# omnirevolve/omnirevolve-image-processor

Measured on NVIDIA B200. Metric: megapixels/sec (resize+color+edge), higher is better.
Workload: dtype u8

## Files before the change

### omnirevolve-image-processor_b200/csrc/label_pipe.cu

```cuda
#include "fast_device.cuh"

#include <algorithm>
#include <vector>
#include <stdio.h>
#include <stdlib.h>
#include <string.h>

#define LP_ZBUF 8192
#define SP_TRY(expr) do { int rc__ = (expr); if (rc__ != OMNI_OK) return rc__; } while (0)


__global__ void __launch_bounds__(256) fk_permute_boxes3(const u8 *__restrict__ boxes, uint2 *__restrict__ boxes3)
{
    const int idx = blockIdx.x * blockDim.x + threadIdx.x;
    if (idx >= RC_COUNT) return;
    const int ci = ((idx & 63) << 12) | (((idx >> 6) & 63) << 6) | (idx >> 12);
    const u8 *q = boxes + 6 * ci;
    boxes3[idx] = make_uint2((u32)q[0] | ((u32)q[1] << 8) | ((u32)q[2] << 16) | ((u32)q[3] << 24), (u32)q[4] | ((u32)q[5] << 8));
}

__device__ __forceinline__ u32 lp_candidates(const AssignParams &P, const float (&lo)[3], const float (&hi)[3], bool &sane)
{
    const int K = P.K;
    float U = 3.0e38f;
// ... 170 lines not shown
            u32 t = nibw & (nibw >> 1) & (nibw >> 2) & (nibw >> 3) & 0x11111111u;
            t = (t | (t >> 3)) & 0x03030303u;
            mm = (t * 0x01041040u) >> 24;
        }
        if (!full) {
            const int nv = max(0, min(8, w - xbase));
            const u32 keep = nv >= 8 ? 0xffffffffu : ((1u << (4 * nv)) - 1u);
            nibw &= keep;
            mm &= (1u << nv) - 1u;
        }
        const int cnt = __popc(mm);
        int x = cnt;
#pragma unroll
        for (int d = 1; d < 32; d <<= 1) {
            int t = __shfl_up_sync(0xffffffffu, x, d);
            if (lane >= d) x += t;
        }
        const int nq = __shfl_sync(0xffffffffu, x, 31);
        if (nq) {
            int pos = x - cnt;
#pragma unroll
            for (int j = 0; j < 8; j++)
                if ((mm >> j) & 1u) sq[pos++] = (u8)(8 * lane + j);
            __syncwarp();
            for (int i = lane; i < nq; i += 32) {
                const int pi = sq[i];
                const u8 *p = spx + 3 * pi;
                int L, a, b, best = 0;
                lab_noclamp(s_gam, s_cbrt, p[0], p[1], p[2], L, a, b);
                u32 mk = __ldg(cells + (((L >> CELL_SHIFT) * CELL_N + (a >> CELL_SHIFT)) * CELL_N + (b >> CELL_SHIFT)));
                const float f0 = (float)L, f1 = (float)a, f2 = (float)b;
                float bd = 3.0e38f;
                do {
                    const int k = __ffs(mk) - 1;
                    mk &= mk - 1u;
                    const float4 ck = s_ctr[k];
                    float d0 = __fsub_rn(f0, ck.x), d1 = __fsub_rn(f1, ck.y), d2 = __fsub_rn(f2, ck.z);
                    float d = __fadd_rn(__fadd_rn(__fmul_rn(d0, d0), __fmul_rn(d1, d1)), __fmul_rn(d2, d2));
                    if (d < bd) { bd = d; best = k; }
                } while (mk);
                slab[pi] = s_lut[best];
            }
            __syncwarp();
            if (mm) {
                const uint2 lb = *reinterpret_cast<const uint2 *>(slab + 8 * lane);
                u32 t0 = lb.x & 0x0F0F0F0Fu, t1 = lb.y & 0x0F0F0F0Fu;
                t0 = (t0 | (t0 >> 4)) & 0x00FF00FFu; t0 = (t0 | (t0 >> 8)) & 0xFFFFu;
                t1 = (t1 | (t1 >> 4)) & 0x00FF00FFu; t1 = (t1 | (t1 >> 8)) & 0xFFFFu;
                const u32 fix = t0 | (t1 << 16);
                u32 m = mm;
                m = (m | (m << 12)) & 0x000F000Fu; m = (m | (m << 6)) & 0x03030303u; m = (m | (m << 3)) & 0x11111111u;
                m *= 15u;
                nibw = (nibw & ~m) | (fix & m);
            }
        }
        if (labels) {
            u32 b0 = nibw & 0xFFFFu, b1 = nibw >> 16;
            b0 = (b0 | (b0 << 8)) & 0x00FF00FFu; b0 = (b0 | (b0 << 4)) & 0x0F0F0F0Fu;
            b1 = (b1 | (b1 << 8)) & 0x00FF00FFu; b1 = (b1 | (b1 << 4)) & 0x0F0F0F0Fu;
            u8 *lrow = labels + (size_t)yy * lpitch + xbase;
            if (lab_vec && xbase + 8 <= w) *reinterpret_cast<uint2 *>(lrow) = make_uint2(b0, b1);
            else
                for (int j = 0; j < 8 && xbase + j < w; j++) lrow[j] = (u8)((nibw >> (4 * j)) & 15u);
        }
        {
            u32 r[4];
#pragma unroll
            for (int b = 0; b < 4; b++) {
                const u32 xb = (nibw >> b) & 0x11111111u;
                const u32 x1 = (xb | (xb >> 3)) & 0x03030303u;
                r[b] = x1 * 0x01041040u;
            }
            const u32 pk = __byte_perm(__byte_perm(r[0], r[1], 0x7373), __byte_perm(r[2], r[3], 0x7373), 0x5410);
            u32 t = __shfl_xor_sync(0xffffffffu, pk, 1);
            const u32 v1 = __byte_perm(pk, t, sel1);
            t = __shfl_xor_sync(0xffffffffu, v1, 2);
            const u32 word = __byte_perm(v1, t, sel2);
            if (c * 8 + (lane >> 2) < ws) slices[(((size_t)f * h + y) * ws + (size_t)c * 8) * 4 + lane] = word;
        }
    }
    if (lane == 0) asm volatile("cp.async.bulk.wait_group.read 0;" ::: "memory");
}

#define LO_WARPS 4
#define LP_COLS 30
#define LO_ROWS 8

__global__ void __launch_bounds__(LO_WARPS * 32) fk_label_open(const uint4 *__restrict__ slices, int ws, size_t plane, int h, int w, int nf,
                                                               u32 *__restrict__ od_out, int strips, int wcols)
{
    const int lane = threadIdx.x & 31;
    const long long gw = (long long)blockIdx.x * LO_WARPS + (threadIdx.x >> 5);
    const long long per_f = (long long)strips * wcols;
    if (gw >= per_f * nf) return;
    const int f = (int)(gw / per_f);
    const int rem = (int)(gw - (long long)f * per_f);
    const int strip = rem / wcols, wx = rem - strip * wcols;
    const int ww = (w + 31) >> 5;
    const int c = wx * LP_COLS - 1 + lane;
    const bool inimg = c >= 0 && c < ww;
    const bool owned = inimg && lane >= 1 && lane <= LP_COLS;
    const u32 cm = inimg ? range_mask(32 * c, w) : 0u;
    const u32 lfix = (c == 0) ? 1u : 0u;
    const u32 rfix = (c == ww - 1) ? (1u << ((w - 1) & 31)) : 0u;
    const uint4 *sl = slices + (size_t)f * plane;
    u32 *od = od_out + (size_t)f * plane;
    const int ys = strip * LO_ROWS, ye = min(h, ys + LO_ROWS);
    u32 sp[4] = {0u, 0u, 0u, 0u}, dh1 = 0u, dh2 = 0u, dv1 = 0u, hu2 = 0u, hu3 = 0u;
    u32 ns[4], ne[4];
    auto fetch = [&](const int r) {
        const bool rin = r >= 0 && r < h;
        uint4 v = make_uint4(0u, 0u, 0u, 0u), ev = v;
        if (rin) {
            const uint4 *row = sl + (size_t)r * ws;
            if (inimg) v = __ldg(row + c);
            if (lane == 0 && c - 1 >= 0 && c - 1 < ww) ev = __ldg(row + c - 1);
            if (lane == 31 && c + 1 >= 0 && c + 1 < ww) ev = __ldg(row + c + 1);
        }
        ns[0] = v.x; ns[1] = v.y; ns[2] = v.z; ns[3] = v.w;
        ne[0] = ev.x; ne[1] = ev.y; ne[2] = ev.z; ne[3] = ev.w;
    };
    fetch(ys - 2);
    for (int r = ys - 2; r < ye + 2; r++) {
        u32 s[4], e[4];
#pragma unroll
        for (int b = 0; b < 4; b++) { s[b] = ns[b]; e[b] = ne[b]; }
        fetch(r + 1);
        const bool rin = r >= 0 && r < h;
        u32 dl = 0u, dr = 0u, dv = 0u;
#pragma unroll
        for (int b = 0; b < 4; b++) {
            const u32 m = s[b];
            u32 l = __shfl_up_sync(0xffffffffu, m, 1), rr = __shfl_down_sync(0xffffffffu, m, 1);
            if (lane == 0) l = e[b];
            if (lane == 31) rr = e[b];
            dl |= m ^ __funnelshift_l(l, m, 1);
            dr |= m ^ __funnelshift_r(m, rr, 1);
            dv |= m ^ sp[b];
            sp[b] = m;
        }
        dl &= ~lfix; dr &= ~rfix;
        const u32 dh0 = rin ? (dl | dr) : 0u;
        const u32 dv0 = (rin && r > 0) ? dv : 0u;
        const bool yin = r - 1 >= 0 && r - 1 < h;
        const u32 U = yin ? (~(dh2 | dh1 | dh0 | dv1 | dv0) & cm) : 0u;
        const u32 l = __shfl_up_sync(0xffffffffu, U, 1), rr = __shfl_down_sync(0xffffffffu, U, 1);
        const u32 hu1 = U | __funnelshift_l(l, U, 1) | __funnelshift_r(U, rr, 1);
        const int z = r - 2;
        if (owned && z >= ys && z < ye) od[(size_t)z * ws + c] = (hu3 | hu2 | hu1) & cm;
        hu3 = hu2; hu2 = hu1; dh2 = dh1; dh1 = dh0; dv1 = dv0;
    }
}

template <int OP>
__device__ __forceinline__ u32 step32(const u32 u, const u32 m, const u32 d)
{
    if (OP == ST_ER || OP == ST_DR) {
        const u32 v = OP == ST_ER ? (u & m & d) : (u | m | d);
        const u32 l = __shfl_up_sync(0xffffffffu, v, 1), r = __shfl_down_sync(0xffffffffu, v, 1);
        const u32 sl = __funnelshift_l(l, v, 1), sr = __funnelshift_r(v, r, 1);
        return OP == ST_ER ? (v & sl & sr) : (v | sl | sr);
    }
    if (OP == ST_EC || OP == ST_DC) {
        const u32 l = __shfl_up_sync(0xffffffffu, m, 1), r = __shfl_down_sync(0xffffffffu, m, 1);
        const u32 sl = __funnelshift_l(l, m, 1), sr = __funnelshift_r(m, r, 1);
        return OP == ST_EC ? ((m & sl & sr) & u & d) : ((m | sl | sr) | u | d);
    }
    return m;
}

template <int NEXT, bool ROWFIX, bool COLFIX>
__device__ __forceinline__ u32 oob_fix32(u32 v, const u32 colvalid, const bool row_inside)
{
    if (NEXT == ST_NONE) return COLFIX ? (v & colvalid) : v;
    if (op_is_erode(NEXT)) {
        if (ROWFIX && !row_inside) return 0xffffffffu;
        return COLFIX ? (v | ~colvalid) : v;
    }
    if (ROWFIX && !row_inside) return 0u;
    return COLFIX ? (v & colvalid) : v;
}

template <u32 CODE, int S>
struct MorphChain32 {
    template <int TAP, bool ROWFIX, bool COLFIX>
    static __device__ __forceinline__ void run(u32 cur, u32 (&p1)[8], u32 (&p2)[8], int t, int h, u32 colvalid, u32 &tap_out, u32 &fin)
    {
        constexpr int N = code_len(CODE);
        if (S == TAP) tap_out = cur;
        if constexpr (S < N) {
            constexpr int OP = code_op(CODE, S);
            constexpr int NEXT = (S + 1 < N) ? code_op(CODE, S + 1) : ST_NONE;
            u32 out = step32<OP>(p2[S], p1[S], cur);
            p2[S] = p1[S]; p1[S] = cur;
            const int r = t - S - 1;
            out = oob_fix32<NEXT, ROWFIX, COLFIX>(out, colvalid, !ROWFIX || (r >= 0 && r < h));
            MorphChain32<CODE, S + 1>::template run<TAP, ROWFIX, COLFIX>(out, p1, p2, t, h, colvalid, tap_out, fin);
        } else {
            fin = cur;
        }
    }
};

#ifndef ML_ORDER
#define ML_ORDER 1
#endif
#ifndef ML_MINB
#define ML_MINB 1
#endif
template <u32 CODE, int TAP, int TR, bool RUNS>
__global__ void __launch_bounds__(128, ML_MINB) fk_morph_lab(const uint4 *__restrict__ slices, const u32 *__restrict__ od, u32 *__restrict__ out_bits, int ws,
                                                    size_t plane, int h, int w, int K, u8 *__restrict__ masks, size_t mstride, size_t mpitch,
                                                    int aligned16, u32 *__restrict__ tap_bits, int wcols, int strips, int n_planes, long long n_units,
                                                    const __grid_constant__ MorphRuns R)
{
    constexpr int N = code_len(CODE);
    constexpr int EXT = RUNS ? 2 : 0;
    constexpr int TILES = TR / ET_R;
    __shared__ uint2 s_lut8[256];
    __shared__ u32 s_item[4][TILES][32];
    expand_lut_init(s_lut8, threadIdx.x, blockDim.x);
    __syncthreads();
    const int lane = threadIdx.x & 31, wid = threadIdx.x >> 5;
    const long long unit = (long long)blockIdx.x * 4 + wid;
    if (unit >= n_units) return;
#if ML_ORDER == 3
    const int p = (int)(unit % n_planes);
    const long long u2 = unit / n_planes;
    const int wx = (int)(u2 % wcols), strip = (int)(u2 / wcols);
#else
    const int wx = (int)(unit % wcols);
    const long long u2 = unit / wcols;
#if ML_ORDER == 1
    const int p = (int)(u2 % n_planes), strip = (int)(u2 / n_planes);
#else
    const int strip = (int)(u2 % strips), p = (int)(u2 / strips);
#endif
#endif
    const int ww = (w + 31) >> 5;
    const int c = wx * LP_COLS - 1 + lane;
    const bool inimg = c >= 0 && c < ww;
    const bool owned = inimg && lane >= 1 && lane <= LP_COLS;
    const int f = p / K, k = p - f * K;
    const int y0 = strip * TR, y1 = min(h, y0 + TR);
    const int t_first = y0 - N - EXT;
    const uint4 *sl = slices + (ptrdiff_t)f * (ptrdiff_t)plane + (ptrdiff_t)t_first * ws + c;
    const u32 *odp = od + (ptrdiff_t)f * (ptrdiff_t)plane + (ptrdiff_t)t_first * ws + c;
    u8 *mrow = masks + (size_t)p * mstride + (ptrdiff_t)(t_first - TAP) * (ptrdiff_t)mpitch;
    u32 *trow = tap_bits + (ptrdiff_t)p * (ptrdiff_t)plane + (ptrdiff_t)(t_first - TAP) * ws + c;
    u32 *frow = out_bits + (ptrdiff_t)p * (ptrdiff_t)plane + (ptrdiff_t)(t_first - N) * ws + c;
    const u32 n0 = (k & 1) ? 0u : 0xffffffffu, n1 = (k & 2) ? 0u : 0xffffffffu, n2 = (k & 4) ? 0u : 0xffffffffu,
              n3 = (k & 8) ? 0u : 0xffffffffu;
    const u32 colvalid = inimg ? range_mask(32 * c, w) : 0u;
    const u32 lv = (c >= 1 && c <= ww) ? 0xC0000000u : 0u;
    const u32 rv = (c + 1 >= 0) ? (range_mask(32 * c + 32, w) & 3u) : 0u;
    constexpr int OP0 = code_op(CODE, 0);
    u32 p1[8], p2[8];
#pragma unroll
    for (int s = 0; s < 8; s++) p1[s] = p2[s] = 0u;
    uint4 nsl = make_uint4(0u, 0u, 0u, 0u);
    u32 nod = 0u;
    auto fetch = [&](const int t) {
        nod = 0u;
        if (t >= 0 && t < h && inimg) { nod = __ldg(odp); nsl = __ldg(sl); }
        odp += ws; sl += ws;
    };
    u32 live1 = 0u, live0 = 0u;
    auto rows = [&](auto rowfix_tag, auto colfix_tag) {
        constexpr bool ROWFIX = decltype(rowfix_tag)::value, COLFIX = decltype(colfix_tag)::value;
        fetch(t_first);
        for (int t = t_first; t < y1 + N + EXT; t++) {
            u32 cur = nod & (nsl.x ^ n0) & (nsl.y ^ n1) & (nsl.z ^ n2) & (nsl.w ^ n3);
            const bool inside = t >= 0 && t < h;
            fetch(t + 1);
            cur = oob_fix32<OP0, ROWFIX, COLFIX>(cur, colvalid, !ROWFIX || inside);
            u32 tap = 0u, fin = 0u;
            MorphChain32<CODE, 0>::template run<TAP, ROWFIX, COLFIX>(cur, p1, p2, t, h, colvalid, tap, fin);
            {
                const int r = t - TAP;
                if (r >= y0 && r < y1 && owned) {
                    if (masks) store_word_bytes_lut(mrow, 32 * c, w, tap, aligned16, s_lut8);
                    if (tap_bits) *trow = tap & colvalid;
                }
                mrow += mpitch; trow += ws;
            }
            if (!RUNS) continue;
            const int r = t - N;
            if (r >= y0 && r < y1 && owned) *frow = fin & colvalid;
            frow += ws;
            if (r >= y0 - 2 && r < y1 + 2 && (!ROWFIX || (r >= 0 && r < h))) {
                const u32 l = __shfl_up_sync(0xffffffffu, fin, 1), rr = __shfl_down_sync(0xffffffffu, fin, 1);
                const bool h1 = ((fin & colvalid) | (l & lv) | (rr & rv)) != 0u, h0 = ((~fin & colvalid) | (~l & lv) | (~rr & rv)) != 0u;
                const int q = r - y0, sub = q & 7;
                u32 m = 1u << ((q >> 3) + 1);
                if (sub < 2) m |= m >> 1;
                if (sub >= 6) m |= m << 1;
                m = (m >> 1) & ((1u << TILES) - 1u);
                if (h1) live1 |= m;
                if (h0) live0 |= m;
            }
        }
    };
    const bool rowfix = !(y0 - N - EXT >= 0 && y1 + N + EXT <= h);
    const bool colfix = __any_sync(0xffffffffu, colvalid != 0xffffffffu);
    if (rowfix) { if (colfix) rows(std::true_type{}, std::true_type{}); else rows(std::true_type{}, std::false_type{}); }
    else { if (colfix) rows(std::false_type{}, std::true_type{}); else rows(std::false_type{}, std::false_type{}); }
    if (!RUNS) return;
    const u32 live = owned ? (live1 & live0) : 0u;
    int n_items = 0, run = 0, run_j0 = 0;
    u32 lens = 0u;
    auto emit = [&]() {
        lens |= (u32)run << (3 * n_items);
        s_item[wid][n_items++][lane] = ((u32)p << 27) | ((u32)run_j0 << 13) | (u32)c;
        run = 0;
    };
#pragma unroll
    for (int tl = 0; tl < TILES; tl++) {
        const int ty0 = y0 + tl * ET_R;
        if (ty0 >= y1) break;
        if ((live >> tl) & 1u) {
            if (run == 0) run_j0 = ty0 / ET_R;
            if (++run == R.maxt) emit();
        } else {
            if (run) emit();
            if (owned && R.zero_fill) {
                const int ty1 = min(y1, ty0 + ET_R);
                for (int y = ty0; y < ty1; y++) {
                    const size_t o = (size_t)p * plane + (size_t)y * ws + c;
                    R.cbits[o] = 0u; R.sbits[o] = 0u;
                    if (R.edges) store_word_bytes(R.edges + (size_t)p * R.estride + (size_t)y * R.epitch, 32 * c, w, 0u, R.aligned16);
                }
            }
        }
    }
    if (run) emit();
#pragma unroll
    for (int nt = 1; nt <= ET_MAXT; nt++) {
        int mine = 0;
        for (int i = 0; i < n_items; i++) mine += ((lens >> (3 * i)) & 7u) == (u32)nt;
        int x = mine;
#pragma unroll
        for (int d = 1; d < 32; d <<= 1) {
            int y = __shfl_up_sync(0xffffffffu, x, d);
            if (lane >= d) x += y;
        }
        const int total = __shfl_sync(0xffffffffu, x, 31);
        if (total == 0) continue;
        int base = 0;
        if (lane == 31) base = atomicAdd(R.run_counts + nt - 1, total);
        base = __shfl_sync(0xffffffffu, base, 31);
        int pos = base + x - mine;
        for (int i = 0; i < n_items; i++)
            if (((lens >> (3 * i)) & 7u) == (u32)nt) R.run_items[R.off.v[nt - 1] + pos++] = s_item[wid][i][lane];
    }
}

#define WS5_LABEL_BYTES ((size_t)CELL_COUNT * sizeof(u32) + RC_NIB_BYTES + RC_MB_BYTES)

static int label_tables(omni_ctx *ctx, const AssignParams &P, u32 **cells, u8 **rtab, cudaStream_t st)
{
    SP_TRY(omni_ws_reserve(ctx, 5, WS5_BYTES + WS5_LABEL_BYTES));
    *cells = (u32 *)((u8 *)ctx->ws[5] + WS5_BYTES);
    *rtab = (u8 *)(*cells + CELL_COUNT);
    if ((ctx->table_cache || ctx->tables_hold) && ctx->cells3_valid && ctx->cells3_ws == ctx->ws[5] && ctx->cells3_stream == (void *)st && ctx->cells3_K == P.K &&
        memcmp(ctx->cells3_c, P.c, sizeof(float) * 3 * P.K) == 0 && memcmp(ctx->cells3_lut, P.lut, P.K) == 0)
        return OMNI_OK;
    memcpy(ctx->cells3_c, P.c, sizeof(float) * 3 * P.K);
    memcpy(ctx->cells3_lut, P.lut, P.K);
    ctx->cells3_K = P.K; ctx->cells3_stream = (void *)st; ctx->cells3_valid = 1; ctx->cells3_ws = ctx->ws[5];
    if (!ctx->d_rgb_boxes3) {
        SP_TRY(fast_rgb_boxes(ctx, st));
        OMNI_CUDA(cudaMalloc(&ctx->d_rgb_boxes3, (size_t)RC_COUNT * sizeof(uint2)));
        KScope ks(ctx, "rgb_boxes", st);
        fk_permute_boxes3<<<RC_COUNT / 256, 256, 0, st>>>(ctx->d_rgb_boxes, (uint2 *)ctx->d_rgb_boxes3);
        OMNI_CUDA(cudaGetLastError());
    }
    KScope ks(ctx, "build_tables", st);
    fk_build_tables3<<<LP_TAB_BLOCKS, 256, 0, st>>>(P, (const uint2 *)ctx->d_rgb_boxes3, *rtab, (u32 *)(*rtab + RC_NIB_BYTES), *cells);
    OMNI_CUDA(cudaGetLastError());
    return OMNI_OK;
}

constexpr u32 CODE_L_N = mk_code(ST_DR, ST_ER);
constexpr u32 CODE_L_O = mk_code(ST_DR, ST_ER, ST_EC, ST_DC);
constexpr u32 CODE_L_C = mk_code(ST_DR, ST_ER, ST_DC, ST_EC);
constexpr u32 CODE_L_OC = mk_code(ST_DR, ST_ER, ST_EC, ST_DC, ST_DC, ST_EC);

static cudaError_t launch_morph_lab(int kind , const uint4 *slices, const u32 *od, u32 *m2, const BitGeom &g, int K, int KT,
                                    u8 *masks, size_t mstride, size_t mpitch, u32 *tap_bits, const MorphRuns &R, cudaStream_t st)
{
    const int wcols = (g.ww + LP_COLS - 1) / LP_COLS;
    const int al = plane_align(masks, mstride, mpitch);
#ifdef ML_TR
    const int tr = ML_TR;
#else
    static int resident = 0;
    if (resident == 0) {
        int per_sm = 0, dev = 0, sms = 0;
        if (cudaOccupancyMaxActiveBlocksPerMultiprocessor(&per_sm, fk_morph_lab<CODE_L_OC, 2, 64, true>, 128, 0) != cudaSuccess || per_sm < 1) per_sm = 4;
        if (cudaGetDevice(&dev) != cudaSuccess || cudaDeviceGetAttribute(&sms, cudaDevAttrMultiProcessorCount, dev) != cudaSuccess || sms < 1) sms = 148;
        cudaGetLastError();
        resident = per_sm * 4 * sms;
    }
    int tr = 32;
    long long best = -1;
    for (int cand : {32, 56, 64}) {
        const long long units = (long long)wcols * ((g.h + cand - 1) / cand) * KT;
        const long long cost = ((units + resident - 1) / resident) * (cand + 20);
        if (best < 0 || cost <= best) { best = cost; tr = cand; }
    }
#endif
    const int strips = (g.h + tr - 1) / tr;
    const long long n_units = (long long)wcols * strips * KT;
    dim3 b(128), grid((unsigned)((n_units + 3) / 4));
#define LL2(CODE, TRV, RUNS) fk_morph_lab<CODE, 2, TRV, RUNS><<<grid, b, 0, st>>>(slices, od, m2, g.ws, g.plane, g.h, g.w, K, masks, mstride, mpitch, al, tap_bits, wcols, strips, KT, n_units, R)
#ifdef ML_TR
#define LL(CODE, RUNS) LL2(CODE, ML_TR, RUNS)
#else
#define LL(CODE, RUNS) do { if (tr == 64) LL2(CODE, 64, RUNS); else if (tr == 56) LL2(CODE, 56, RUNS); else LL2(CODE, 32, RUNS); } while (0)
#endif
    switch (kind) {
    case -1: LL(CODE_L_N, false); break;
    case 0: LL(CODE_L_N, true); break;
    case 1: LL(CODE_L_O, true); break;
    case 2: LL(CODE_L_C, true); break;
    default: LL(CODE_L_OC, true); break;
    }
#undef LL
#undef LL2
    return cudaGetLastError();
}

struct LabelPlanes { u32 *slices, *mask_bits, *edge_bits, *cand_bits; };

static int label_pipeline(omni_ctx *ctx, const u8 *d_bgr, int nf, size_t frame_stride, int h, int w, size_t pitch, const AssignParams &P,
                          const omni_edge_params *prm, int low, int high, u8 *d_labels, size_t lpitch,
                          u8 *d_masks, size_t m_plane, size_t mpitch, u8 *d_edges, size_t e_plane, size_t epitch, bool want_mask_bits,
                          cudaStream_t st, LabelPlanes *out, bool skip_hysteresis = false )
{
    const int K = P.K, KT = nf * K;
    const int kind = prm ? morph03_kind(prm) : -1;
    if (prm && (low < 0 || kind < 0 || prm->ksize != 3)) return OMNI_ERR_UNSUPPORTED;
    if (K > RC_MAX_K || KT > OMNI_MAX_K || !lut_below_k(P) || !edges3_sparse_ok(h, w, KT)) return OMNI_ERR_UNSUPPORTED;
    const BitGeom g = make_geom(h, w);
    if ((long long)nf * h * ((w + 255) >> 8) >= (1ll << 30)) return OMNI_ERR_UNSUPPORTED;
    OMNI_CUDA(fast_tables());
    const size_t pbytes = g.plane * sizeof(u32);
    auto al = [](size_t v) { return (v + 255) & ~(size_t)255; };
    const size_t o_sl = 0, o_od = al(o_sl + pbytes * 4 * nf), o_m2 = al(o_od + pbytes * nf), o_s = al(o_m2 + pbytes * KT),
                 o_c = o_s + al(pbytes * KT), o_mb = al(o_c + pbytes * KT), bits_total = al(o_mb + (want_mask_bits ? pbytes * KT : 0));
    SP_TRY(omni_ws_reserve(ctx, 4, bits_total));
    u8 *b4 = (u8 *)ctx->ws[4];
    u32 *slices = (u32 *)(b4 + o_sl), *od = (u32 *)(b4 + o_od), *M2 = (u32 *)(b4 + o_m2), *sbits = (u32 *)(b4 + o_s), *cbits = (u32 *)(b4 + o_c);
    u32 *mbits = want_mask_bits ? (u32 *)(b4 + o_mb) : nullptr;
    if (out) { out->slices = slices; out->mask_bits = mbits; out->edge_bits = prm ? sbits : nullptr; out->cand_bits = prm ? cbits : nullptr; }
    MorphRuns R{};
    bool sparse = false;
    ZeroJob Z{};
    if (prm) {
        SP_TRY(edge_pass_begin(ctx, g, KT, sbits, cbits, d_edges, e_plane, epitch, st, &R, &sparse, d_edges != nullptr, d_edges ? &Z : nullptr));
        if (!sparse) return OMNI_ERR_UNSUPPORTED;
    }
    u32 *cells = nullptr;
    u8 *rtab = nullptr;
    SP_TRY(label_tables(ctx, P, &cells, &rtab, st));
    const u16 *labtab = fast_lab_table();
    if (!labtab) { omni_set_error("Lab tables not available"); return OMNI_ERR_CUDA; }
    {
        if (!ctx->occ_assign_sl) {
            OMNI_CUDA(cudaFuncSetAttribute(fk_assign_slices<true>, cudaFuncAttributeMaxDynamicSharedMemorySize, RA_SMEM + LP_ZBUF));
            OMNI_CUDA(cudaFuncSetAttribute(fk_assign_slices<false>, cudaFuncAttributeMaxDynamicSharedMemorySize, RA_SMEM + LP_ZBUF));
            ctx->occ_assign_sl = 1;
        }
        const long long chunks = (long long)nf * h * ((w + 255) >> 8);
        const int grid = (int)std::max<long long>(1, std::min<long long>(persist_blocks(ctx, 1), (chunks + RA_WARPS - 1) / RA_WARPS));
        for (int z = 0; z < 2; z++)
            Z.per[z] = (unsigned)(((Z.n16[z] + (unsigned long long)chunks - 1) / (unsigned long long)chunks + 31) & ~31ull);
        KScope ks(ctx, "assign_bits", st);
        if (K >= 16)
            fk_assign_slices<true><<<grid, RA_THREADS, RA_SMEM + LP_ZBUF, st>>>(d_bgr, h, w, pitch, P, (const uint4 *)rtab, cells, labtab, d_labels,
                                                                                lpitch, slices, g.ws, nf, frame_stride, Z);
        else
            fk_assign_slices<false><<<grid, RA_THREADS, RA_SMEM + LP_ZBUF, st>>>(d_bgr, h, w, pitch, P, (const uint4 *)rtab, cells, labtab, d_labels,
                                                                                 lpitch, slices, g.ws, nf, frame_stride, Z);
        OMNI_CUDA(cudaGetLastError());
    }
    {
        const int wcols = (g.ww + LP_COLS - 1) / LP_COLS, strips = (h + LO_ROWS - 1) / LO_ROWS;
        const long long warps = (long long)nf * strips * wcols;
        KScope ks(ctx, "label_open", st);
        fk_label_open<<<(unsigned)((warps + LO_WARPS - 1) / LO_WARPS), LO_WARPS * 32, 0, st>>>((const uint4 *)slices, g.ws, g.plane, h, w, nf, od, strips,
                                                                                              wcols);
        OMNI_CUDA(cudaGetLastError());
    }
    OMNI_LAUNCH(ctx, st, "morph_bits", launch_morph_lab(kind, (const uint4 *)slices, od, M2, g, K, KT, d_masks, m_plane, mpitch, mbits, R, st));
    if (!prm) return OMNI_OK;
    if (ctx->edge_join) {
        OMNI_CUDA(cudaStreamWaitEvent(st, ctx->edge_join, 0));
        ctx->edge_join = nullptr;
    }
    const int al16 = plane_align(d_edges, e_plane, epitch);
    OMNI_LAUNCH(ctx, st, "edges3_bits", launch_edges3_sparse(M2, g.ws, g.plane, h, w, KT, low, high, persist_blocks(ctx, ctx->e3s_per_sm),
                                                             sbits, cbits, d_edges, e_plane, epitch, al16, ctx->d_flags + 4,
                                                             (u32 *)ctx->ws[5] + HYST_WL_OFFSET, HY_WL_CAP, ctx->d_flags + 16,
                                                             ctx->d_flags + 20, (const u32 *)ctx->ws[6], st));
    if (skip_hysteresis) return OMNI_OK;
    return run_hysteresis(ctx, sbits, cbits, g, KT, d_edges, e_plane, epitch, st);
}

void label_ws_bytes(int h, int w, int K, int nf, size_t out[OMNI_WS_SLOTS])
{
    const BitGeom g = make_geom(h, w);
    const int KT = nf * K;
    const size_t pbytes = g.plane * sizeof(u32);
    auto al = [](size_t v) { return (v + 255) & ~(size_t)255; };
    const size_t o_od = al(pbytes * 4 * nf), o_m2 = al(o_od + pbytes * nf), o_s = al(o_m2 + pbytes * KT), o_c = o_s + al(pbytes * KT),
                 o_mb = al(o_c + pbytes * KT);
    unsigned off[ET_MAXT];
    out[4] = std::max(out[4], al(o_mb + pbytes * KT));
    out[5] = std::max(out[5], WS5_BYTES + WS5_LABEL_BYTES);
    out[6] = std::max(out[6], edges3_run_words(h, w, KT, off) * sizeof(u32));
}

int sparse_color_edge(omni_ctx *ctx, const u8 *d_bgr, int nf, size_t frame_stride, int h, int w, size_t pitch, const AssignParams &P,
                      const omni_edge_params *prm, int low, int high, u8 *d_labels, size_t lpitch,
                      u8 *d_masks, size_t m_plane, size_t mpitch, u8 *d_edges, size_t e_plane, size_t epitch, cudaStream_t st)
{
    return label_pipeline(ctx, d_bgr, nf, frame_stride, h, w, pitch, P, prm, low, high, d_labels, lpitch, d_masks, m_plane, mpitch, d_edges,
                          e_plane, epitch, false, st, nullptr);
}

__global__ void __launch_bounds__(256) fk_pack_planes(const u32 *__restrict__ src, int ws, size_t plane, int K, int h, int w,
                                                      u8 *__restrict__ dst, size_t dplane, size_t dpitch, int msb_first,
                                                      unsigned long long *__restrict__ counts)
{
    const int ww = (w + 31) >> 5, rb = (w + 7) >> 3;
    const int lane = threadIdx.x & 31, k = blockIdx.y;
    const int warps = (int)gridDim.x * (int)(blockDim.x >> 5);
    if (k >= K) return;
    const u32 *sp = src + (size_t)k * plane;
    u8 *dp = dst + (size_t)k * dplane;
    const bool aligned = (((uintptr_t)dp | dpitch) & 3) == 0;
    unsigned n = 0;
    for (int y = (int)blockIdx.x * (int)(blockDim.x >> 5) + (int)(threadIdx.x >> 5); y < h; y += warps) {
        const u32 *srow = sp + (size_t)y * ws;
        u8 *row = dp + (size_t)y * dpitch;
        for (int c = lane; c < ww; c += 32) {
            const u32 word = srow[c] & range_mask(32 * c, w);
            const u32 o = msb_first ? __byte_perm(__brev(word), 0u, 0x0123) : word;
            if (aligned && 4 * c + 4 <= rb) *reinterpret_cast<u32 *>(row + 4 * c) = o;
            else
                for (int i = 0; 4 * c + i < rb && i < 4; i++) row[4 * c + i] = (u8)(o >> (8 * i));
            n += (unsigned)__popc(word);
        }
    }
    if (counts) {
#pragma unroll
        for (int d = 16; d > 0; d >>= 1) n += __shfl_xor_sync(0xffffffffu, n, d);
        if (lane == 0 && n) atomicAdd(counts + k, (unsigned long long)n);
    }
}

static inline dim3 pack_grid(int blocks, int K, int h)
{
    const int per_plane = std::max(1, std::min((h + 7) / 8, (blocks + K - 1) / K));
    return dim3((unsigned)per_plane, (unsigned)K);
}

__global__ void __launch_bounds__(256) fk_unpack_planes(const u8 *__restrict__ src, size_t splane, size_t spitch, int msb_first, int K, int h, int w,
                                                        u32 *__restrict__ dst, int ws, size_t plane)
{
    const int rb = (w + 7) >> 3;
    const long long total = (long long)K * h * ws;
    for (long long u = (long long)blockIdx.x * blockDim.x + threadIdx.x; u < total; u += (long long)gridDim.x * blockDim.x) {
        const int c = (int)(u % ws);
        const long long r2 = u / ws;
        const int y = (int)(r2 % h), k = (int)(r2 / h);
        const u8 *row = src + (size_t)k * splane + (size_t)y * spitch + 4 * c;
        u32 v = 0u;
        for (int i = 0; i < 4 && 4 * c + i < rb; i++) v |= (u32)row[i] << (8 * i);
        if (msb_first) v = __brev(__byte_perm(v, 0u, 0x0123));
        dst[(size_t)k * plane + (size_t)y * ws + c] = v & range_mask(32 * c, w);
    }
}

cudaError_t launch_unpack_planes(const u8 *src, size_t splane, size_t spitch, int msb_first, int K, int h, int w, u32 *dst, int ws,
                                 size_t plane, int blocks, cudaStream_t st)
{
    fk_unpack_planes<<<blocks, 256, 0, st>>>(src, splane, spitch, msb_first, K, h, w, dst, ws, plane);
    return cudaGetLastError();
}
cudaError_t launch_pack_planes(const u32 *src, int ws, size_t plane, int K, int h, int w, u8 *dst, size_t dplane, size_t dpitch, int msb_first,
                               int blocks, cudaStream_t st)
{
    fk_pack_planes<<<pack_grid(blocks, K, h), 256, 0, st>>>(src, ws, plane, K, h, w, dst, dplane, dpitch, msb_first, nullptr);
    return cudaGetLastError();
}

__global__ void __launch_bounds__(256) fk_count_labels_sl(const uint4 *__restrict__ slices, int ws, int h, int w, int K,
                                                          unsigned long long *__restrict__ counts)
// ... 375 lines not shown
```

Before: 42910.

## Fuse label-open mask into morph kernel with TMA-staged shared-memory tiles

Removes the separate label_open kernel and its global od buffer. The morph kernel now bulk-copies slice rows into shared memory with mbarrier-tracked cp.async.bulk, computes the open mask per block into shared memory, and lets each warp process one of up to eight labels of the same frame from the shared tile. Run items move from shared memory into registers. This saves one launch plus a global write and read of od and repeated slice reads across labels. The cost is redundant halo recomputation, a larger dynamic shared-memory footprint that may lower occupancy, and a smaller block size when K is small.

Result: faster. 45910, median of 6 (+7.0%).

```diff
diff --git a/omnirevolve-image-processor_b200/csrc/label_pipe.cu b/omnirevolve-image-processor_b200/csrc/label_pipe.cu
--- a/omnirevolve-image-processor_b200/csrc/label_pipe.cu
+++ b/omnirevolve-image-processor_b200/csrc/label_pipe.cu
@@ -276,75 +276,12 @@
     if (lane == 0) asm volatile("cp.async.bulk.wait_group.read 0;" ::: "memory");
 }
 
-#define LO_WARPS 4
 #define LP_COLS 30
-#define LO_ROWS 8
-
-__global__ void __launch_bounds__(LO_WARPS * 32) fk_label_open(const uint4 *__restrict__ slices, int ws, size_t plane, int h, int w, int nf,
-                                                               u32 *__restrict__ od_out, int strips, int wcols)
-{
-    const int lane = threadIdx.x & 31;
-    const long long gw = (long long)blockIdx.x * LO_WARPS + (threadIdx.x >> 5);
-    const long long per_f = (long long)strips * wcols;
-    if (gw >= per_f * nf) return;
-    const int f = (int)(gw / per_f);
-    const int rem = (int)(gw - (long long)f * per_f);
-    const int strip = rem / wcols, wx = rem - strip * wcols;
-    const int ww = (w + 31) >> 5;
-    const int c = wx * LP_COLS - 1 + lane;
-    const bool inimg = c >= 0 && c < ww;
-    const bool owned = inimg && lane >= 1 && lane <= LP_COLS;
-    const u32 cm = inimg ? range_mask(32 * c, w) : 0u;
-    const u32 lfix = (c == 0) ? 1u : 0u;
-    const u32 rfix = (c == ww - 1) ? (1u << ((w - 1) & 31)) : 0u;
-    const uint4 *sl = slices + (size_t)f * plane;
-    u32 *od = od_out + (size_t)f * plane;
-    const int ys = strip * LO_ROWS, ye = min(h, ys + LO_ROWS);
-    u32 sp[4] = {0u, 0u, 0u, 0u}, dh1 = 0u, dh2 = 0u, dv1 = 0u, hu2 = 0u, hu3 = 0u;
-    u32 ns[4], ne[4];
-    auto fetch = [&](const int r) {
-        const bool rin = r >= 0 && r < h;
-        uint4 v = make_uint4(0u, 0u, 0u, 0u), ev = v;
-        if (rin) {
-            const uint4 *row = sl + (size_t)r * ws;
-            if (inimg) v = __ldg(row + c);
-            if (lane == 0 && c - 1 >= 0 && c - 1 < ww) ev = __ldg(row + c - 1);
-            if (lane == 31 && c + 1 >= 0 && c + 1 < ww) ev = __ldg(row + c + 1);
-        }
-        ns[0] = v.x; ns[1] = v.y; ns[2] = v.z; ns[3] = v.w;
-        ne[0] = ev.x; ne[1] = ev.y; ne[2] = ev.z; ne[3] = ev.w;
-    };
-    fetch(ys - 2);
-    for (int r = ys - 2; r < ye + 2; r++) {
-        u32 s[4], e[4];
-#pragma unroll
-        for (int b = 0; b < 4; b++) { s[b] = ns[b]; e[b] = ne[b]; }
-        fetch(r + 1);
-        const bool rin = r >= 0 && r < h;
-        u32 dl = 0u, dr = 0u, dv = 0u;
-#pragma unroll
-        for (int b = 0; b < 4; b++) {
-            const u32 m = s[b];
-            u32 l = __shfl_up_sync(0xffffffffu, m, 1), rr = __shfl_down_sync(0xffffffffu, m, 1);
-            if (lane == 0) l = e[b];
-            if (lane == 31) rr = e[b];
-            dl |= m ^ __funnelshift_l(l, m, 1);
-            dr |= m ^ __funnelshift_r(m, rr, 1);
-            dv |= m ^ sp[b];
-            sp[b] = m;
-        }
-        dl &= ~lfix; dr &= ~rfix;
-        const u32 dh0 = rin ? (dl | dr) : 0u;
-        const u32 dv0 = (rin && r > 0) ? dv : 0u;
-        const bool yin = r - 1 >= 0 && r - 1 < h;
-        const u32 U = yin ? (~(dh2 | dh1 | dh0 | dv1 | dv0) & cm) : 0u;
-        const u32 l = __shfl_up_sync(0xffffffffu, U, 1), rr = __shfl_down_sync(0xffffffffu, U, 1);
-        const u32 hu1 = U | __funnelshift_l(l, U, 1) | __funnelshift_r(U, rr, 1);
-        const int z = r - 2;
-        if (owned && z >= ys && z < ye) od[(size_t)z * ws + c] = (hu3 | hu2 | hu1) & cm;
-        hu3 = hu2; hu2 = hu1; dh2 = dh1; dh1 = dh0; dv1 = dv0;
-    }
-}
+#define OM_SCOLS 34
+#define OM_CHUNK 8
+#ifndef OM_PMAX
+#define OM_PMAX 8
+#endif
 
 template <int OP>
 __device__ __forceinline__ u32 step32(const u32 u, const u32 m, const u32 d)
@@ -396,77 +333,155 @@
     }
 };
 
-#ifndef ML_ORDER
-#define ML_ORDER 1
-#endif
-#ifndef ML_MINB
-#define ML_MINB 1
-#endif
+template <u32 CODE, int TR, bool RUNS>
+struct OmLayout {
+    static constexpr int N = code_len(CODE), EXT = RUNS ? 2 : 0;
+    static constexpr int RS = TR + 2 * (N + EXT + 2);
+    static constexpr int RO = TR + 2 * (N + EXT);
+    static constexpr int NBAR = (RS + OM_CHUNK - 1) / OM_CHUNK;
+    static constexpr int TILES = TR / ET_R;
+    static constexpr size_t OFF_OD = (size_t)RS * OM_SCOLS * sizeof(uint4);
+    static constexpr size_t bytes() { return OFF_OD + (size_t)(RO + 1) * 32 * sizeof(u32); }
+};
+
+__device__ __forceinline__ void om_wait(u32 bar)
+{
+    u32 done = 0;
+    while (!done)
+        asm volatile("{\n\t.reg .pred p;\n\tmbarrier.try_wait.parity.shared::cta.b64 p, [%1], 0;\n\tselp.u32 %0, 1, 0, p;\n\t}"
+                     : "=r"(done) : "r"(bar) : "memory");
+}
+
 template <u32 CODE, int TAP, int TR, bool RUNS>
-__global__ void __launch_bounds__(128, ML_MINB) fk_morph_lab(const uint4 *__restrict__ slices, const u32 *__restrict__ od, u32 *__restrict__ out_bits, int ws,
-                                                    size_t plane, int h, int w, int K, u8 *__restrict__ masks, size_t mstride, size_t mpitch,
-                                                    int aligned16, u32 *__restrict__ tap_bits, int wcols, int strips, int n_planes, long long n_units,
-                                                    const __grid_constant__ MorphRuns R)
-{
-    constexpr int N = code_len(CODE);
-    constexpr int EXT = RUNS ? 2 : 0;
-    constexpr int TILES = TR / ET_R;
+__global__ void __launch_bounds__(OM_PMAX * 32) fk_open_morph(const uint4 *__restrict__ slices, u32 *__restrict__ out_bits, int ws, size_t plane,
+                                                             int h, int w, int K, int P, int groups, int nf, u8 *__restrict__ masks,
+                                                             size_t mstride, size_t mpitch, int aligned16, u32 *__restrict__ tap_bits,
+                                                             int wcols, const __grid_constant__ MorphRuns R)
+{
+    using L = OmLayout<CODE, TR, RUNS>;
+    constexpr int N = L::N, EXT = L::EXT, TILES = L::TILES;
+    extern __shared__ __align__(16) u8 smem[];
+    uint4 *s_sl = reinterpret_cast<uint4 *>(smem);
+    u32 *s_od = reinterpret_cast<u32 *>(smem + L::OFF_OD);
     __shared__ uint2 s_lut8[256];
-    __shared__ u32 s_item[4][TILES][32];
+    __shared__ __align__(8) unsigned long long s_bar[L::NBAR];
+    const int lane = threadIdx.x & 31, wid = threadIdx.x >> 5;
+    const int wx = (int)(blockIdx.x % (unsigned)wcols);
+    const int u2 = (int)(blockIdx.x / (unsigned)wcols);
+    const int fg = u2 % (nf * groups), strip = u2 / (nf * groups);
+    const int f = fg / groups, grp = fg - f * groups;
+    const int ww = (w + 31) >> 5;
+    const int c = wx * LP_COLS - 1 + lane;
+    const int cs = c - lane - 1;
+    const int lo = max(0, -cs), hi = min(OM_SCOLS, ww - cs);
+    const int y0 = strip * TR, y1 = min(h, y0 + TR);
+    const int ys0 = y0 - N - EXT - 2, rs = y1 - y0 + 2 * (N + EXT + 2);
+    const int yo0 = y0 - N - EXT, ro = y1 - y0 + 2 * (N + EXT);
+    const u32 bar0 = (u32)__cvta_generic_to_shared(s_bar);
+    if (threadIdx.x == 0) {
+        for (int j = 0; j < L::NBAR; j++) asm volatile("mbarrier.init.shared::cta.b64 [%0], 1;" ::"r"(bar0 + 8u * j));
+        asm volatile("fence.mbarrier_init.release.cluster;" ::: "memory");
+        const uint4 *src = slices + (size_t)f * plane + cs + lo;
+        const u32 dst0 = (u32)__cvta_generic_to_shared(s_sl + lo), bytes = (u32)(hi - lo) * 16u;
+        for (int j = 0; j * OM_CHUNK < rs; j++) {
+            const int a = max(j * OM_CHUNK, -ys0), b = min(min(rs, (j + 1) * OM_CHUNK), h - ys0);
+            asm volatile("mbarrier.arrive.expect_tx.shared::cta.b64 _, [%0], %1;" ::"r"(bar0 + 8u * j), "r"(b > a ? (u32)(b - a) * bytes : 0u)
+                         : "memory");
+            for (int r = a; r < b; r++)
+                asm volatile("cp.async.bulk.shared::cluster.global.mbarrier::complete_tx::bytes [%0], [%1], %2, [%3];"
+                             ::"r"(dst0 + (u32)(r * OM_SCOLS * 16)), "l"(src + (ptrdiff_t)(ys0 + r) * ws), "r"(bytes), "r"(bar0 + 8u * j)
+                             : "memory");
+        }
+    }
+    for (int i = threadIdx.x; i < rs * OM_SCOLS; i += blockDim.x) {
+        const int r = i / OM_SCOLS, col = i - r * OM_SCOLS, y = ys0 + r;
+        if (y < 0 || y >= h || col < lo || col >= hi) s_sl[i] = make_uint4(0u, 0u, 0u, 0u);
+    }
     expand_lut_init(s_lut8, threadIdx.x, blockDim.x);
     __syncthreads();
-    const int lane = threadIdx.x & 31, wid = threadIdx.x >> 5;
-    const long long unit = (long long)blockIdx.x * 4 + wid;
-    if (unit >= n_units) return;
-#if ML_ORDER == 3
-    const int p = (int)(unit % n_planes);
-    const long long u2 = unit / n_planes;
-    const int wx = (int)(u2 % wcols), strip = (int)(u2 / wcols);
-#else
-    const int wx = (int)(unit % wcols);
-    const long long u2 = unit / wcols;
-#if ML_ORDER == 1
-    const int p = (int)(u2 % n_planes), strip = (int)(u2 / n_planes);
-#else
-    const int strip = (int)(u2 % strips), p = (int)(u2 / strips);
-#endif
-#endif
-    const int ww = (w + 31) >> 5;
-    const int c = wx * LP_COLS - 1 + lane;
     const bool inimg = c >= 0 && c < ww;
+    const u32 colvalid = inimg ? range_mask(32 * c, w) : 0u;
+    {
+        const int seg = (ro + P - 1) / P;
+        const int ys = yo0 + wid * seg, ye = min(yo0 + ro, ys + seg);
+        if (ys < ye) {
+            const int ra = ys - 2 - ys0, rb = ye + 2 - ys0;
+            for (int j = ra / OM_CHUNK; j * OM_CHUNK < rb; j++) om_wait(bar0 + 8u * j);
+            const int ce = lane == 0 ? c - 1 : c + 1;
+            const u32 cme = (ce >= 0 && ce < ww) ? range_mask(32 * ce, w) : 0u;
+            const u32 lfix = (c == 0) ? 1u : 0u, lfixe = (ce == 0) ? 1u : 0u;
+            const u32 rlast = 1u << ((w - 1) & 31);
+            const u32 rfix = (c == ww - 1) ? rlast : 0u, rfixe = (ce == ww - 1) ? rlast : 0u;
+            const int eidx = lane == 0 ? 0 : OM_SCOLS - 1;
+            u32 sp[4] = {0u, 0u, 0u, 0u}, spe[4] = {0u, 0u, 0u, 0u};
+            u32 dh1 = 0u, dh2 = 0u, dv1 = 0u, hu2 = 0u, hu3 = 0u, dhe1 = 0u, dhe2 = 0u, dve1 = 0u;
+            for (int r = ys - 2; r < ye + 2; r++) {
+                const uint4 *row = s_sl + (r - ys0) * OM_SCOLS;
+                const uint4 v = row[lane + 1], ev = row[eidx];
+                const u32 s[4] = {v.x, v.y, v.z, v.w}, e[4] = {ev.x, ev.y, ev.z, ev.w};
+                const bool rin = r >= 0 && r < h;
+                u32 dl = 0u, dr = 0u, dv = 0u, dle = 0u, dre = 0u, dve = 0u;
+#pragma unroll
+                for (int b = 0; b < 4; b++) {
+                    const u32 m = s[b], x = e[b];
+                    u32 l = __shfl_up_sync(0xffffffffu, m, 1), rr = __shfl_down_sync(0xffffffffu, m, 1);
+                    if (lane == 0) l = x;
+                    if (lane == 31) rr = x;
+                    dl |= m ^ __funnelshift_l(l, m, 1);
+                    dr |= m ^ __funnelshift_r(m, rr, 1);
+                    dv |= m ^ sp[b];
+                    sp[b] = m;
+                    dle |= x ^ (lane == 0 ? (x << 1) : __funnelshift_l(m, x, 1));
+                    dre |= x ^ (lane == 0 ? __funnelshift_r(x, m, 1) : (x >> 1));
+                    dve |= x ^ spe[b];
+                    spe[b] = x;
+                }
+                dl &= ~lfix; dr &= ~rfix; dle &= ~lfixe; dre &= ~rfixe;
+                const u32 dh0 = rin ? (dl | dr) : 0u, dhe0 = rin ? (dle | dre) : 0u;
+                const u32 dv0 = (rin && r > 0) ? dv : 0u, dve0 = (rin && r > 0) ? dve : 0u;
+                const bool yin = r - 1 >= 0 && r - 1 < h;
+                const u32 U = yin ? (~(dh2 | dh1 | dh0 | dv1 | dv0) & colvalid) : 0u;
+                const u32 Ue = yin ? (~(dhe2 | dhe1 | dhe0 | dve1 | dve0) & cme) : 0u;
+                u32 l = __shfl_up_sync(0xffffffffu, U, 1), rr = __shfl_down_sync(0xffffffffu, U, 1);
+                if (lane == 0) l = Ue;
+                if (lane == 31) rr = Ue;
+                const u32 hu1 = U | __funnelshift_l(l, U, 1) | __funnelshift_r(U, rr, 1);
+                const int z = r - 2;
+                if (z >= ys) s_od[(z - yo0) * 32 + lane] = (z >= 0 && z < h) ? ((hu3 | hu2 | hu1) & colvalid) : 0u;
+                hu3 = hu2; hu2 = hu1; dh2 = dh1; dh1 = dh0; dv1 = dv0; dhe2 = dhe1; dhe1 = dhe0; dve1 = dve0;
+            }
+        }
+    }
+    __syncthreads();
+    const int k = grp * P + wid;
+    if (k >= K) return;
+    const int p = f * K + k;
     const bool owned = inimg && lane >= 1 && lane <= LP_COLS;
-    const int f = p / K, k = p - f * K;
-    const int y0 = strip * TR, y1 = min(h, y0 + TR);
     const int t_first = y0 - N - EXT;
-    const uint4 *sl = slices + (ptrdiff_t)f * (ptrdiff_t)plane + (ptrdiff_t)t_first * ws + c;
-    const u32 *odp = od + (ptrdiff_t)f * (ptrdiff_t)plane + (ptrdiff_t)t_first * ws + c;
     u8 *mrow = masks + (size_t)p * mstride + (ptrdiff_t)(t_first - TAP) * (ptrdiff_t)mpitch;
     u32 *trow = tap_bits + (ptrdiff_t)p * (ptrdiff_t)plane + (ptrdiff_t)(t_first - TAP) * ws + c;
     u32 *frow = out_bits + (ptrdiff_t)p * (ptrdiff_t)plane + (ptrdiff_t)(t_first - N) * ws + c;
     const u32 n0 = (k & 1) ? 0u : 0xffffffffu, n1 = (k & 2) ? 0u : 0xffffffffu, n2 = (k & 4) ? 0u : 0xffffffffu,
               n3 = (k & 8) ? 0u : 0xffffffffu;
-    const u32 colvalid = inimg ? range_mask(32 * c, w) : 0u;
     const u32 lv = (c >= 1 && c <= ww) ? 0xC0000000u : 0u;
     const u32 rv = (c + 1 >= 0) ? (range_mask(32 * c + 32, w) & 3u) : 0u;
     constexpr int OP0 = code_op(CODE, 0);
     u32 p1[8], p2[8];
 #pragma unroll
     for (int s = 0; s < 8; s++) p1[s] = p2[s] = 0u;
-    uint4 nsl = make_uint4(0u, 0u, 0u, 0u);
-    u32 nod = 0u;
-    auto fetch = [&](const int t) {
-        nod = 0u;
-        if (t >= 0 && t < h && inimg) { nod = __ldg(odp); nsl = __ldg(sl); }
-        odp += ws; sl += ws;
-    };
+    const uint4 *ssl = s_sl + (t_first - ys0) * OM_SCOLS + lane + 1;
+    const u32 *sod = s_od + lane;
+    uint4 nsl;
+    u32 nod;
+    auto fetch = [&]() { nsl = *ssl; nod = *sod; ssl += OM_SCOLS; sod += 32; };
     u32 live1 = 0u, live0 = 0u;
     auto rows = [&](auto rowfix_tag, auto colfix_tag) {
         constexpr bool ROWFIX = decltype(rowfix_tag)::value, COLFIX = decltype(colfix_tag)::value;
-        fetch(t_first);
+        fetch();
         for (int t = t_first; t < y1 + N + EXT; t++) {
             u32 cur = nod & (nsl.x ^ n0) & (nsl.y ^ n1) & (nsl.z ^ n2) & (nsl.w ^ n3);
             const bool inside = t >= 0 && t < h;
-            fetch(t + 1);
+            fetch();
             cur = oob_fix32<OP0, ROWFIX, COLFIX>(cur, colvalid, !ROWFIX || inside);
             u32 tap = 0u, fin = 0u;
             MorphChain32<CODE, 0>::template run<TAP, ROWFIX, COLFIX>(cur, p1, p2, t, h, colvalid, tap, fin);
@@ -500,12 +515,13 @@
     if (rowfix) { if (colfix) rows(std::true_type{}, std::true_type{}); else rows(std::true_type{}, std::false_type{}); }
     else { if (colfix) rows(std::false_type{}, std::true_type{}); else rows(std::false_type{}, std::false_type{}); }
     if (!RUNS) return;
+    u32 item[TILES + 1];
     const u32 live = owned ? (live1 & live0) : 0u;
-    int n_items = 0, run = 0, run_j0 = 0;
+    int run = 0, run_j0 = 0;
     u32 lens = 0u;
-    auto emit = [&]() {
-        lens |= (u32)run << (3 * n_items);
-        s_item[wid][n_items++][lane] = ((u32)p << 27) | ((u32)run_j0 << 13) | (u32)c;
+    auto emit = [&](const int slot) {
+        lens |= (u32)run << (3 * slot);
+        item[slot] = ((u32)p << 27) | ((u32)run_j0 << 13) | (u32)c;
         run = 0;
     };
 #pragma unroll
@@ -514,9 +530,9 @@
         if (ty0 >= y1) break;
         if ((live >> tl) & 1u) {
             if (run == 0) run_j0 = ty0 / ET_R;
-            if (++run == R.maxt) emit();
+            if (++run == R.maxt) emit(tl);
         } else {
-            if (run) emit();
+            if (run) emit(tl);
             if (owned && R.zero_fill) {
                 const int ty1 = min(y1, ty0 + ET_R);
                 for (int y = ty0; y < ty1; y++) {
@@ -527,11 +543,12 @@
             }
         }
     }
-    if (run) emit();
+    if (run) emit(TILES);
 #pragma unroll
     for (int nt = 1; nt <= ET_MAXT; nt++) {
         int mine = 0;
-        for (int i = 0; i < n_items; i++) mine += ((lens >> (3 * i)) & 7u) == (u32)nt;
+#pragma unroll
+        for (int i = 0; i <= TILES; i++) mine += ((lens >> (3 * i)) & 7u) == (u32)nt;
         int x = mine;
 #pragma unroll
         for (int d = 1; d < 32; d <<= 1) {
@@ -544,8 +561,9 @@
         if (lane == 31) base = atomicAdd(R.run_counts + nt - 1, total);
         base = __shfl_sync(0xffffffffu, base, 31);
         int pos = base + x - mine;
-        for (int i = 0; i < n_items; i++)
-            if (((lens >> (3 * i)) & 7u) == (u32)nt) R.run_items[R.off.v[nt - 1] + pos++] = s_item[wid][i][lane];
+#pragma unroll
+        for (int i = 0; i <= TILES; i++)
+            if (((lens >> (3 * i)) & 7u) == (u32)nt) R.run_items[R.off.v[nt - 1] + pos++] = item[i];
     }
 }
 
@@ -580,34 +598,59 @@
 constexpr u32 CODE_L_C = mk_code(ST_DR, ST_ER, ST_DC, ST_EC);
 constexpr u32 CODE_L_OC = mk_code(ST_DR, ST_ER, ST_EC, ST_DC, ST_DC, ST_EC);
 
-static cudaError_t launch_morph_lab(int kind , const uint4 *slices, const u32 *od, u32 *m2, const BitGeom &g, int K, int KT,
-                                    u8 *masks, size_t mstride, size_t mpitch, u32 *tap_bits, const MorphRuns &R, cudaStream_t st)
-{
+template <u32 CODE, int TR, bool RUNS>
+static cudaError_t open_morph_smem_attr()
+{
+    static unsigned done = 0;
+    int dev = 0;
+    if (cudaGetDevice(&dev) != cudaSuccess) return cudaGetLastError();
+    if (dev < 32 && ((done >> dev) & 1u)) return cudaSuccess;
+    const cudaError_t e = cudaFuncSetAttribute(fk_open_morph<CODE, 2, TR, RUNS>, cudaFuncAttributeMaxDynamicSharedMemorySize,
+                                               (int)OmLayout<CODE, TR, RUNS>::bytes());
+    if (e == cudaSuccess && dev < 32) done |= 1u << dev;
+    return e;
+}
+
+static cudaError_t launch_open_morph(int kind , const uint4 *slices, u32 *m2, const BitGeom &g, int K, int nf,
+                                     u8 *masks, size_t mstride, size_t mpitch, u32 *tap_bits, const MorphRuns &R, cudaStream_t st)
+{
+    const int KT = nf * K;
     const int wcols = (g.ww + LP_COLS - 1) / LP_COLS;
     const int al = plane_align(masks, mstride, mpitch);
+    const int groups = (K + OM_PMAX - 1) / OM_PMAX, P = (K + groups - 1) / groups;
 #ifdef ML_TR
     const int tr = ML_TR;
 #else
-    static int resident = 0;
-    if (resident == 0) {
-        int per_sm = 0, dev = 0, sms = 0;
-        if (cudaOccupancyMaxActiveBlocksPerMultiprocessor(&per_sm, fk_morph_lab<CODE_L_OC, 2, 64, true>, 128, 0) != cudaSuccess || per_sm < 1) per_sm = 4;
+    static int resident[OM_PMAX + 1][3] = {};
+    const int cands[3] = {32, 56, 64};
+    if (resident[P][0] == 0) {
+        int dev = 0, sms = 0;
         if (cudaGetDevice(&dev) != cudaSuccess || cudaDeviceGetAttribute(&sms, cudaDevAttrMultiProcessorCount, dev) != cudaSuccess || sms < 1) sms = 148;
+        auto occ = [&](auto kern, cudaError_t attr, size_t smem) {
+            int per_sm = 0;
+            if (attr != cudaSuccess || cudaOccupancyMaxActiveBlocksPerMultiprocessor(&per_sm, kern, 32 * P, smem) != cudaSuccess || per_sm < 1) per_sm = 1;
+            return per_sm * P * sms;
+        };
+        resident[P][0] = occ(fk_open_morph<CODE_L_OC, 2, 32, true>, open_morph_smem_attr<CODE_L_OC, 32, true>(), OmLayout<CODE_L_OC, 32, true>::bytes());
+        resident[P][1] = occ(fk_open_morph<CODE_L_OC, 2, 56, true>, open_morph_smem_attr<CODE_L_OC, 56, true>(), OmLayout<CODE_L_OC, 56, true>::bytes());
+        resident[P][2] = occ(fk_open_morph<CODE_L_OC, 2, 64, true>, open_morph_smem_attr<CODE_L_OC, 64, true>(), OmLayout<CODE_L_OC, 64, true>::bytes());
         cudaGetLastError();
-        resident = per_sm * 4 * sms;
     }
     int tr = 32;
     long long best = -1;
-    for (int cand : {32, 56, 64}) {
+    for (int i = 0; i < 3; i++) {
+        const int cand = cands[i], res = resident[P][i];
         const long long units = (long long)wcols * ((g.h + cand - 1) / cand) * KT;
-        const long long cost = ((units + resident - 1) / resident) * (cand + 20);
+        const long long cost = ((units + res - 1) / res) * (cand + 20);
         if (best < 0 || cost <= best) { best = cost; tr = cand; }
     }
 #endif
     const int strips = (g.h + tr - 1) / tr;
-    const long long n_units = (long long)wcols * strips * KT;
-    dim3 b(128), grid((unsigned)((n_units + 3) / 4));
-#define LL2(CODE, TRV, RUNS) fk_morph_lab<CODE, 2, TRV, RUNS><<<grid, b, 0, st>>>(slices, od, m2, g.ws, g.plane, g.h, g.w, K, masks, mstride, mpitch, al, tap_bits, wcols, strips, KT, n_units, R)
+    const dim3 grid((unsigned)((long long)wcols * groups * nf * strips)), b(32 * P);
+    cudaError_t e = cudaSuccess;
+#define LL2(CODE, TRV, RUNS) do { if ((e = open_morph_smem_attr<CODE, TRV, RUNS>()) != cudaSuccess) return e; \
+        fk_open_morph<CODE, 2, TRV, RUNS><<<grid, b, OmLayout<CODE, TRV, RUNS>::bytes(), st>>>(slices, m2, g.ws, g.plane, g.h, g.w, K, P, groups, nf, \
+                                                 masks, mstride, mpitch, al, tap_bits, wcols, R); } while (0)
 #ifdef ML_TR
 #define LL(CODE, RUNS) LL2(CODE, ML_TR, RUNS)
 #else
@@ -641,11 +684,11 @@
     OMNI_CUDA(fast_tables());
     const size_t pbytes = g.plane * sizeof(u32);
     auto al = [](size_t v) { return (v + 255) & ~(size_t)255; };
-    const size_t o_sl = 0, o_od = al(o_sl + pbytes * 4 * nf), o_m2 = al(o_od + pbytes * nf), o_s = al(o_m2 + pbytes * KT),
+    const size_t o_sl = 0, o_m2 = al(o_sl + pbytes * 4 * nf), o_s = al(o_m2 + pbytes * KT),
                  o_c = o_s + al(pbytes * KT), o_mb = al(o_c + pbytes * KT), bits_total = al(o_mb + (want_mask_bits ? pbytes * KT : 0));
     SP_TRY(omni_ws_reserve(ctx, 4, bits_total));
     u8 *b4 = (u8 *)ctx->ws[4];
-    u32 *slices = (u32 *)(b4 + o_sl), *od = (u32 *)(b4 + o_od), *M2 = (u32 *)(b4 + o_m2), *sbits = (u32 *)(b4 + o_s), *cbits = (u32 *)(b4 + o_c);
+    u32 *slices = (u32 *)(b4 + o_sl), *M2 = (u32 *)(b4 + o_m2), *sbits = (u32 *)(b4 + o_s), *cbits = (u32 *)(b4 + o_c);
     u32 *mbits = want_mask_bits ? (u32 *)(b4 + o_mb) : nullptr;
     if (out) { out->slices = slices; out->mask_bits = mbits; out->edge_bits = prm ? sbits : nullptr; out->cand_bits = prm ? cbits : nullptr; }
     MorphRuns R{};
@@ -679,15 +722,7 @@
                                                                                  lpitch, slices, g.ws, nf, frame_stride, Z);
         OMNI_CUDA(cudaGetLastError());
     }
-    {
-        const int wcols = (g.ww + LP_COLS - 1) / LP_COLS, strips = (h + LO_ROWS - 1) / LO_ROWS;
-        const long long warps = (long long)nf * strips * wcols;
-        KScope ks(ctx, "label_open", st);
-        fk_label_open<<<(unsigned)((warps + LO_WARPS - 1) / LO_WARPS), LO_WARPS * 32, 0, st>>>((const uint4 *)slices, g.ws, g.plane, h, w, nf, od, strips,
-                                                                                              wcols);
-        OMNI_CUDA(cudaGetLastError());
-    }
-    OMNI_LAUNCH(ctx, st, "morph_bits", launch_morph_lab(kind, (const uint4 *)slices, od, M2, g, K, KT, d_masks, m_plane, mpitch, mbits, R, st));
+    OMNI_LAUNCH(ctx, st, "morph_bits", launch_open_morph(kind, (const uint4 *)slices, M2, g, K, nf, d_masks, m_plane, mpitch, mbits, R, st));
     if (!prm) return OMNI_OK;
     if (ctx->edge_join) {
         OMNI_CUDA(cudaStreamWaitEvent(st, ctx->edge_join, 0));
@@ -708,8 +743,7 @@
     const int KT = nf * K;
     const size_t pbytes = g.plane * sizeof(u32);
     auto al = [](size_t v) { return (v + 255) & ~(size_t)255; };
-    const size_t o_od = al(pbytes * 4 * nf), o_m2 = al(o_od + pbytes * nf), o_s = al(o_m2 + pbytes * KT), o_c = o_s + al(pbytes * KT),
-                 o_mb = al(o_c + pbytes * KT);
+    const size_t o_m2 = al(pbytes * 4 * nf), o_s = al(o_m2 + pbytes * KT), o_c = o_s + al(pbytes * KT), o_mb = al(o_c + pbytes * KT);
     unsigned off[ET_MAXT];
     out[4] = std::max(out[4], al(o_mb + pbytes * KT));
     out[5] = std::max(out[5], WS5_BYTES + WS5_LABEL_BYTES);
```
